# HuiGuanLab/Lite-MKD

Hardware: AMD Instinct MI355X
Metric: episodes/sec (5-way 5-shot, 8x224^2 frames) (higher is better)
Workload: dtype f32

## Files before the change

### include/lmkd.h

```cpp
#ifndef LMKD_H
#define LMKD_H
#ifdef __cplusplus
extern "C" {
#endif

int lmkd_abi_version(void);
const char* lmkd_last_error(void);
int lmkd_device_check(int device);
int lmkd_set_activation_dtype(int mode);
int lmkd_get_activation_dtype(void);

int lmkd_gemm_f32(char layA, char layB, int M, int N, int K, float alpha, const float* A, long lda, long sA,
                  const float* B, long ldb, long sB, float beta, float* C, long ldc, long sC, const float* bias,
                  int relu, int batch, void* stream);
int lmkd_gemm_set_mode(int mode);
int lmkd_gemm_set_tile(int t);
long lmkd_gemm_ticket_words(void);
int lmkd_gemm_f32_splitk(char layA, char layB, int M, int N, int K, float alpha, const float* A, long lda, long sA,
                         const float* B, long ldb, long sB, float beta, float* C, long ldc, long sC, const float* bias,
                         int relu, int batch, void* workspace, long ws_bytes, unsigned* tickets, void* stream);

long lmkd_conv2d_packed_weight_elems(int Cout, int Cin, int Cs, int KH, int KW, int mode);
int lmkd_conv2d_pack_weights(const float* w_oihw, float* wp, int Cout, int Cin, int Cs, int KH, int KW, int mode ,
                             void* stream);
// ... 175 lines not shown

int lmkd_conv2d_fwd_row_tiles_seg(int N, int H, int W, int Cs, int Cout, int KH, int KW, int stride, int pad, int seg_n0, int* tiles0 );
int lmkd_conv2d_fwd_seg(const float* x, const float* pre_stats , const float* wp, float* y,
                        float* stat_partial, int N, int H, int W, int Cs, int Cout, int KH, int KW, int stride, int pad, int seg_n0, void* stream,
                        const lmkd_amax_desc* amax );
int lmkd_conv2d_bwd_data_bn_tiles_seg(int N, int H, int W, int Cin, int Cout, int KH, int KW, int stride, int pad, int seg_n0, int* tiles0 );
int lmkd_conv2d_bwd_data_seg(const float* dy, const float* wd, float* dx, const float* bn_x ,
                             const float* bn_stats, float* part, int N, int H, int W, int Cin, int Cout, int KH, int KW, int stride, int pad,
                             int accumulate, int seg_n0, void* stream, const lmkd_amax_desc* amax );
long lmkd_conv2d_bwd_weight_workspace_seg(int N, int H, int W, int Cs, int Cout, int KH, int KW, int stride, int pad, int seg_n0);
int lmkd_conv2d_bwd_weight_seg(const float* x, const float* pre_stats , const float* dy, float* dw_oihw, float* workspace,
                               long ws_bytes, int N, int H, int W, int Cs, int Cin, int Cout, int KH, int KW, int stride, int pad, int accumulate,
                               int seg_n0, void* stream, const lmkd_amax_desc* amax );
int lmkd_bn_finalize_seg(const float* partial, int T, int T0, int C, long count0, long count1, const float* gamma, const float* beta, float eps,
                         float* stats , double* scratch, unsigned* tickets, void* stream, const lmkd_amax_desc* amax );
int lmkd_bn_apply_seg(const float* x, const float* stats, const float* res, const float* rstats, float* y, long rows, long rows0, int C, int relu,
                      int res_mode, unsigned* mask_bits, void* stream, const lmkd_amax_desc* amax );
int lmkd_bn_backward_seg(const float* dy, const float* x, const float* yact, const float* stats, const float* gamma, float* dx, float* g_out,
                         float* dgamma, float* dbeta, float* coef, void* workspace, unsigned* tickets, long rows, long rows0, int C, int mask_mode,
                         int accumulate_param_grads, void* stream, const lmkd_amax_desc* amax );
int lmkd_bn_backward_part_seg(const float* part, int T, int T0, const float* dy, const float* x, const float* stats, const float* gamma, float* dx,
                              float* dgamma, float* dbeta, float* coef, void* workspace, unsigned* tickets, long rows, long rows0, int C,
                              int accumulate_param_grads, void* stream, const lmkd_amax_desc* amax );
int lmkd_bn_relu_maxpool_fwd_seg(const float* x, const float* stats, float* y, unsigned char* idx, float* cmax, int N, int N0, int H, int W, int C,
                                 void* stream, const lmkd_amax_desc* amax );
int lmkd_bn_backward_stats_seg(const float* dy, const float* cmax, const float* stats, const float* gamma, float* coef, void* workspace,
                               unsigned* tickets, long pooled_rows, long pooled_rows0, long count, long count0, int C, void* stream);
int lmkd_stem_unpool_bn_bwd_seg(const float* dy, const unsigned char* idx, const float* c, const float* stats, const float* coef, float* dc,
                                float* dgamma, float* dbeta, int accumulate_param_grads, int N, int N0, int H, int W, int C, void* stream,
                                const lmkd_amax_desc* amax );

int lmkd_strm_patchpool_fwd(const float* x, const float* pe, const float* mask, float* y, unsigned char* idx, int F, int H, int W, int C,
                            void* stream);
int lmkd_strm_patchpool_bwd(const float* dy, const float* mask, const unsigned char* idx, float* dx, int F, int H, int W, int C, void* stream);
int lmkd_strm_attn_fwd(const float* x, const float* qkv, const float* gamma, float* y, float* probs, int F, int C, void* stream);
int lmkd_strm_attn_bwd(const float* dy, const float* qkv, const float* probs, const float* gamma, float* dqkv, float* dgamma_part,
                       float* dgamma, int F, int C, void* stream);
long lmkd_strm_tokmlp_parts(long V, int D);
int lmkd_strm_tokmlp_fwd(const float* x, const float* pe, const float* mask, const float* w1, const float* b1, const float* w2, const float* b2,
                         float* xp, float* y, unsigned char* hmask, int V, int L, int D, void* stream);
int lmkd_strm_tokmlp_bwd(const float* dy, const float* xp, const float* mask, const float* w1, const float* b1, const float* w2, float* dx,
                         float* part, float* dparams, int V, int L, int D, void* stream);
int lmkd_strm_pair_embed(const float* P, const float* bias, float* E, int NV, int L, int Hd, void* stream);
int lmkd_strm_patchdist_fwd(const float* E, const int* order, float* dist, int* idx, float* logits, int Ns, int Nq, int way, int shot, int L,
                            int Hd, void* stream);
int lmkd_strm_patchdist_bwd(const float* E, const int* order, const int* pos, const float* dist, const int* idx, const float* g, float* dpre,
// ... 7 lines not shown
```

### lite-mkd_amd/csrc/norm_pool.hip

```cpp
#include "common.h"
#include <vector>
#include <cmath>
#include <algorithm>

#define NP_THREADS 256
static int g_ew_wg_per_cu = 4;
extern "C" int lmkd_set_elementwise_wg_per_cu(int n) {
  LMKD_REQUIRE(n >= 1 && n <= 8, "lmkd_set_elementwise_wg_per_cu: %d outside 1..8 (the BatchNorm partial buffers hold 2048 rows)", n);
  g_ew_wg_per_cu = n;
  return LMKD_OK;
}
static inline int ew_grid(long n_items) {
  long g = (n_items + NP_THREADS - 1) / NP_THREADS;
  if (g > 256 * g_ew_wg_per_cu) g = 256 * g_ew_wg_per_cu;
  if (g < 1) g = 1;
  return (int)g;
}

extern "C" long lmkd_amax_words(void) { return 2 * LMKD_AMAX_SEG_WORDS; }
static inline unsigned* amd_out(const lmkd_amax_desc* d) { return d ? (unsigned*)d->out_words : nullptr; }
static inline const unsigned* amd_ref(const lmkd_amax_desc* d) { return (d && d->out_words) ? (const unsigned*)d->ref_words : nullptr; }

#define LMKD_FENCE_MAX 128
struct FenceArgs { const unsigned* w[LMKD_FENCE_MAX]; unsigned* r[LMKD_FENCE_MAX]; };
// ... 591 lines not shown
      const float4 g = bn_masked_grad<T>(dv[u], xv[u], yact, i0 + u, stats, C, c + 4 * u, mask_mode);
      s1[u].x += g.x; s1[u].y += g.y; s1[u].z += g.z; s1[u].w += g.w;
      s2[u].x = fmaf(g.x, (xv[u].x - mean[u].x) * istd[u].x, s2[u].x); s2[u].y = fmaf(g.y, (xv[u].y - mean[u].y) * istd[u].y, s2[u].y);
      s2[u].z = fmaf(g.z, (xv[u].z - mean[u].z) * istd[u].z, s2[u].z); s2[u].w = fmaf(g.w, (xv[u].w - mean[u].w) * istd[u].w, s2[u].w);
    }
  }
#pragma unroll
  for (int u = 0; u < U; ++u) {
    float* d = sm + ((long)rl * CC + cq * 4 * U + 4 * u) * 2;
    d[0] = s1[u].x; d[1] = s2[u].x; d[2] = s1[u].y; d[3] = s2[u].y; d[4] = s1[u].z; d[5] = s2[u].z; d[6] = s1[u].w; d[7] = s2[u].w;
  }
  __syncthreads();
  for (int j = threadIdx.x; j < 2 * CC; j += NP_THREADS) {
#pragma unroll
    for (int h = 0; h < U; ++h) {
      if (blockIdx.x * U + h >= nbv) break;
      float s = 0.f;
      for (int q = h * RL1; q < (h + 1) * RL1; ++q) s += sm[(long)q * 2 * CC + j];
      partial[(long)(blockIdx.x * U + h) * 2 * C + 2 * c0 + j] = s;
    }
  }
}

struct CoefSeg { int T1; long pstride; double count1; int S0, S1; };
__global__ void bn_bwd_coef_kernel(const float* __restrict__ part, int T, int C, double count, const float* __restrict__ gamma,
                                   const float* __restrict__ stats, float* __restrict__ coef, float* __restrict__ dgamma,
                                   float* __restrict__ dbeta, int accumulate, double* __restrict__ scratch, unsigned* __restrict__ tickets,
                                   CoefSeg cs) {
  __shared__ double sm[CS_LANES][CS_COLS];
  __shared__ double tot[CS_COLS];
  __shared__ int s_last;
  int S = 0;
  const bool seg = gridDim.z > 1;
  if (seg) {
    if (blockIdx.z) { part += cs.pstride; T = cs.T1; count = cs.count1; stats += 5 * C; coef += 5 * C; scratch += (long)(CS_MAX_SLICES + 2) * 2 * C; tickets += LMKD_TICKET_WORDS / 2; S = cs.S1; }
    else S = cs.S0;
  }
  if (!colsum_ticket(part, T, 2 * C, scratch, tickets, sm, tot, &s_last, nullptr, S)) return;
  const int c = blockIdx.x * (CS_COLS / 2) + threadIdx.x;
  if (threadIdx.y != 0 || threadIdx.x >= CS_COLS / 2 || c >= C) return;
  const double sg = tot[2 * threadIdx.x], sgx = tot[2 * threadIdx.x + 1];
  const float g = gamma ? gamma[c] : 1.f;
  const float invstd = stats[C + c];
  coef[c] = g * invstd;
  coef[C + c] = (float)(sg / count);
  coef[2 * C + c] = (float)(sgx / count);
  if (seg) {
    coef[3 * C + c] = (float)sgx;
    coef[4 * C + c] = (float)sg;
    return;
  }
  if (dgamma) dgamma[c] = accumulate ? dgamma[c] + (float)sgx : (float)sgx;
  if (dbeta) dbeta[c] = accumulate ? dbeta[c] + (float)sg : (float)sg;
}

struct ParamGradSeg { float* dgamma; float* dbeta; int accumulate; };
__device__ __forceinline__ void bn_param_grads_seg(const float* __restrict__ coef, int C, const ParamGradSeg& pg) {
  if (blockIdx.x != 0 || !pg.dgamma) return;
  for (int c = threadIdx.x; c < C; c += blockDim.x) {
    const float gx = coef[3 * C + c] + coef[5 * C + 3 * C + c], g = coef[4 * C + c] + coef[5 * C + 4 * C + c];
    pg.dgamma[c] = pg.accumulate ? pg.dgamma[c] + gx : gx;
    if (pg.dbeta) pg.dbeta[c] = pg.accumulate ? pg.dbeta[c] + g : g;
  }
}

template <typename T>
__global__ void bn_bwd_apply_kernel(const T* __restrict__ dy, const T* __restrict__ x, const T* __restrict__ yact,
                                    const float* __restrict__ stats, const float* __restrict__ coef, T* __restrict__ dx,
                                    T* __restrict__ g_out, long n4, int C, int mask_mode, long n4_0, ParamGradSeg pg,
                                    unsigned* __restrict__ amax, const unsigned* __restrict__ aref) {
  constexpr int U = ActU<T>::U;
  const int C4 = C >> 2;
  const long nu = n4 / U;
  if (n4_0 < n4) bn_param_grads_seg(coef, C, pg);
  AmaxStat am = {0.f, 0.f, 0u}, am1 = {0.f, 0.f, 0u};
  const AmaxRef rf0 = amax_ref(aref ? amax_read(aref, 0) : 0u), rf1 = amax_ref(aref ? amax_read(aref, 1) : 0u);
  for (long iu = (long)blockIdx.x * blockDim.x + threadIdx.x; iu < nu; iu += (long)gridDim.x * blockDim.x) {
    float4 xv[U], dv[U], o[U], gq[U];
    ldv<T, U>(x, iu, xv);
    ldv<T, U>(dy, iu, dv);
    const int so = iu * U >= n4_0 ? 5 * C : 0;
// ... 5 lines not shown
      const int c = (int)(i % C4) * 4;
      const float4 g = bn_masked_grad<T>(dv[u], xv[u], yact, i, st, C, c, mask_mode);
      const float4 mean = *reinterpret_cast<const float4*>(st + c);
      const float4 istd = *reinterpret_cast<const float4*>(st + C + c);
      const float4 A = *reinterpret_cast<const float4*>(cf + c);
      const float4 mg = *reinterpret_cast<const float4*>(cf + C + c);
      const float4 mgx = *reinterpret_cast<const float4*>(cf + 2 * C + c);
      o[u].x = A.x * (g.x - mg.x - (xv[u].x - mean.x) * istd.x * mgx.x);
      o[u].y = A.y * (g.y - mg.y - (xv[u].y - mean.y) * istd.y * mgx.y);
      o[u].z = A.z * (g.z - mg.z - (xv[u].z - mean.z) * istd.z * mgx.z);
      o[u].w = A.w * (g.w - mg.w - (xv[u].w - mean.w) * istd.w * mgx.w);
      gq[u] = g;
      if (so) amax_stat4(am1, o[u], rf1); else amax_stat4(am, o[u], rf0);
    }
    stv<T, U>(dx, iu, o);
    if (g_out) stv<T, U>(g_out, iu, gq);
  }
  if (amax) {
    amax_commit_stat(amax, am, aref != nullptr);
    if (n4_0 < n4) amax_commit_stat(amax + LMKD_AMAX_SEG_WORDS, am1, aref != nullptr);
  }
}

extern "C" long lmkd_bn_bwd_workspace(int C) { return (long)(2048 * 2 * C) * sizeof(float) + (long)(66 * 2 * C) * sizeof(double) + 64; }

static int bn_bwd_stats_impl(const float* dy, const float* x, const float* yact, const float* stats, const float* gamma, float* dgamma,
                             float* dbeta, float* coef, void* workspace, unsigned* tickets, long rows, long count, int C, int mask_mode,
                             int accumulate_param_grads, hipStream_t s, const char* who, long rows0 = 0, long count0 = 0) {
  LMKD_REQUIRE(dy && x && stats && coef && workspace && tickets, "%s: null pointer", who);
  const bool seg = rows0 > 0 && rows0 < rows;
  LMKD_REQUIRE(!seg || cdiv(2 * C, CS_COLS) <= LMKD_TICKET_WORDS / 2, "%s: C=%d exceeds the ticket buffer", who, C);
  const int CC = C > 1024 ? 1024 : C;
  const int U = g_lmkd_act_bf16 ? 2 : 1;
  LMKD_REQUIRE(C % (4 * U) == 0 && C % CC == 0 && 256 % (CC / 4) == 0, "%s: unsupported channel count %d", who, C);
  LMKD_REQUIRE((mask_mode != 1 && mask_mode != 3) || yact, "%s: mask_mode 1 / 3 needs the activation output / its bit mask", who);
  LMKD_REQUIRE(mask_mode != 3 || C % 32 == 0, "%s: bit masks need C %% 32 == 0", who);
  LMKD_REQUIRE(cdiv(2 * C, CS_COLS) <= LMKD_TICKET_WORDS, "%s: C=%d exceeds the ticket buffer", who, C);
  const int RL1 = NP_THREADS / (CC / 4), RL = RL1 * U;
  auto blocks = [&](long r) {
    int nb = cdiv(r, (long)RL1 * 8);
    if (nb > 256 * g_ew_wg_per_cu * 2) nb = 256 * g_ew_wg_per_cu * 2;
    if (nb > 2048) nb = 2048;
    return nb < 1 ? 1 : nb;
  };
  const int nb = blocks(seg ? rows0 : rows), nb1 = seg ? blocks(rows - rows0) : 0;
  const int nbx = std::max(nb, nb1);
  float* partial = (float*)workspace;
  double* dscr = (double*)((char*)workspace + (((long)(seg ? 2 : 1) * 2048 * 2 * C * sizeof(float) + 63) / 64) * 64);
  BnSeg bs;
  bs.rows0 = seg ? rows0 : rows; bs.nb1 = nb1;
  const int gz = seg ? 2 : 1;
  if (g_lmkd_act_bf16)
    hipLaunchKernelGGL(bn_bwd_reduce_kernel<lmkd_bf16_t>, dim3(cdiv(nbx, 2), C / CC, gz), dim3(NP_THREADS), (size_t)RL * CC * 2 * sizeof(float), s,
                       (const lmkd_bf16_t*)dy, (const lmkd_bf16_t*)x, (const lmkd_bf16_t*)yact, stats, partial, rows, C, CC, mask_mode, nb, bs);
  else
    hipLaunchKernelGGL(bn_bwd_reduce_kernel<float>, dim3(nbx, C / CC, gz), dim3(NP_THREADS), (size_t)RL * CC * 2 * sizeof(float), s, dy, x, yact,
                       stats, partial, rows, C, CC, mask_mode, nb, bs);
  LMKD_CHECK_LAUNCH("bn_bwd_reduce_kernel");
  CoefSeg cs;
  cs.T1 = nb1; cs.pstride = (long)2048 * 2 * C; cs.count1 = (double)(count - count0); cs.S0 = cs_slices(nb); cs.S1 = seg ? cs_slices(nb1) : 0;
  hipLaunchKernelGGL(bn_bwd_coef_kernel, dim3(cdiv(2 * C, CS_COLS), std::max(cs.S0, cs.S1), gz), dim3(CS_COLS, CS_LANES), 0, s, (const float*)partial, nb, C,
                     (double)(seg ? count0 : count), gamma, stats, coef, dgamma, dbeta, accumulate_param_grads, dscr, tickets, cs);
  LMKD_CHECK_LAUNCH("bn_bwd_coef_kernel");
  return LMKD_OK;
}

extern "C" int lmkd_bn_backward_seg(const float* dy, const float* x, const float* yact, const float* stats, const float* gamma, float* dx,
                                    float* g_out, float* dgamma, float* dbeta, float* coef, void* workspace, unsigned* tickets, long rows,
                                    long rows0, int C, int mask_mode, int accumulate_param_grads, void* stream, const lmkd_amax_desc* amd);
extern "C" int lmkd_bn_backward(const float* dy, const float* x, const float* yact, const float* stats, const float* gamma,
                                float* dx, float* g_out, float* dgamma, float* dbeta, float* coef, void* workspace, unsigned* tickets,
// ... 2 lines not shown
                              accumulate_param_grads, stream, nullptr);
}
extern "C" int lmkd_bn_backward_seg(const float* dy, const float* x, const float* yact, const float* stats, const float* gamma, float* dx,
                                    float* g_out, float* dgamma, float* dbeta, float* coef, void* workspace, unsigned* tickets, long rows,
                                    long rows0, int C, int mask_mode, int accumulate_param_grads, void* stream, const lmkd_amax_desc* amd) {
  unsigned* amax = amd_out(amd);
  const unsigned* aref = amd_ref(amd);
  LMKD_REQUIRE(dx, "lmkd_bn_backward: null pointer");
  hipStream_t s = (hipStream_t)stream;
  if (rows0 <= 0 || rows0 >= rows) rows0 = rows;
  const int rc = bn_bwd_stats_impl(dy, x, yact, stats, gamma, dgamma, dbeta, coef, workspace, tickets, rows, rows, C, mask_mode,
                                   accumulate_param_grads, s, "lmkd_bn_backward", rows0, rows0);
  if (rc) return rc;
  const long n4 = rows * C / 4, n4_0 = rows0 * C / 4;
  ParamGradSeg pg;
  pg.dgamma = dgamma; pg.dbeta = dbeta; pg.accumulate = accumulate_param_grads;
  if (g_lmkd_act_bf16)
    hipLaunchKernelGGL(bn_bwd_apply_kernel<lmkd_bf16_t>, dim3(ew_grid(n4)), dim3(NP_THREADS), 0, s, (const lmkd_bf16_t*)dy, (const lmkd_bf16_t*)x,
                       (const lmkd_bf16_t*)yact, stats, (const float*)coef, (lmkd_bf16_t*)dx, (lmkd_bf16_t*)g_out, n4, C, mask_mode, n4_0, pg, amax, aref);
  else
    hipLaunchKernelGGL(bn_bwd_apply_kernel<float>, dim3(ew_grid(n4)), dim3(NP_THREADS), 0, s, dy, x, yact, stats, (const float*)coef, dx, g_out,
                       n4, C, mask_mode, n4_0, pg, amax, aref);
  LMKD_CHECK_LAUNCH("bn_bwd_apply_kernel");
  return LMKD_OK;
}

extern "C" int lmkd_bn_backward_part_seg(const float* part, int T, int T0, const float* dy, const float* x, const float* stats, const float* gamma,
                                         float* dx, float* dgamma, float* dbeta, float* coef, void* workspace, unsigned* tickets, long rows,
                                         long rows0, int C, int accumulate_param_grads, void* stream, const lmkd_amax_desc* amd);
extern "C" int lmkd_bn_backward_part(const float* part, int T, const float* dy, const float* x, const float* stats, const float* gamma,
                                     float* dx, float* dgamma, float* dbeta, float* coef, void* workspace, unsigned* tickets, long rows, int C,
                                     int accumulate_param_grads, void* stream) {
  return lmkd_bn_backward_part_seg(part, T, T, dy, x, stats, gamma, dx, dgamma, dbeta, coef, workspace, tickets, rows, rows, C,
                                   accumulate_param_grads, stream, nullptr);
}
extern "C" int lmkd_bn_backward_part_seg(const float* part, int T, int T0, const float* dy, const float* x, const float* stats, const float* gamma,
                                         float* dx, float* dgamma, float* dbeta, float* coef, void* workspace, unsigned* tickets, long rows,
                                         long rows0, int C, int accumulate_param_grads, void* stream, const lmkd_amax_desc* amd) {
  unsigned* amax = amd_out(amd);
  const unsigned* aref = amd_ref(amd);
  LMKD_REQUIRE(part && T > 0 && dy && x && stats && dx && coef && workspace && tickets, "lmkd_bn_backward_part: null pointer");
  LMKD_REQUIRE(!g_lmkd_act_bf16 && C % 4 == 0, "lmkd_bn_backward_part: fp32 tensors, C %% 4 == 0");
  const bool seg = T0 > 0 && T0 < T && rows0 > 0 && rows0 < rows;
  LMKD_REQUIRE(seg || (T0 == T && rows0 == rows), "lmkd_bn_backward_part_seg: T0 / rows0 must both name a split or both the whole");
  LMKD_REQUIRE(cdiv(2 * C, CS_COLS) <= LMKD_TICKET_WORDS / (seg ? 2 : 1), "lmkd_bn_backward_part: C=%d exceeds the ticket buffer", C);
  hipStream_t s = (hipStream_t)stream;
// ... 401 lines not shown
```

### lite-mkd_amd/ops.py

```python
import ctypes
import os
import math

import torch

from ._lib import lib
from . import _audit


def _raw_stream(device_index=None):
    return torch._C._cuda_getCurrentRawStream(torch._C._cuda_getDevice() if device_index is None else device_index)


def _stream():
    return ctypes.c_void_p(_raw_stream())


def _p(t):
    if t is None:
        return None
    if _audit.ON:
        _audit.note(t)
    return ctypes.c_void_p(t.data_ptr())

# ... 81 lines not shown
        e = _GEMM_WS[key] = (torch.empty(32 << 20, dtype=torch.uint8, device=like.device),
                             torch.zeros(lib().value("lmkd_gemm_ticket_words"), dtype=torch.int32, device=like.device))
    return e


def stack_rows(a, b):
    if (a.dim() == 2 and b.dim() == 2 and a.shape[1] == b.shape[1] and a.dtype == b.dtype and a.is_contiguous() and b.is_contiguous()
            and a.numel() > 0 and b.numel() > 0 and a.untyped_storage().data_ptr() == b.untyped_storage().data_ptr()
            and a.storage_offset() + a.numel() == b.storage_offset()):
        return torch.as_strided(a, (a.shape[0] + b.shape[0], a.shape[1]), (a.shape[1], 1), a.storage_offset())
    return torch.cat([a, b], 0)


def linear_fwd(x, w, b):
    M, K = x.shape
    N = w.shape[0]
    y = _empty((M, N), x)
    return gemm("K", "K", M, N, K, x, K, w, K, y, N, bias=b)


_TICKETS = {}


def _tickets(like):
    key = (like.device.index, _raw_stream(like.device.index))
    t = _TICKETS.get(key)
    if t is None:
        t = _TICKETS[key] = torch.zeros(lib().value("lmkd_ticket_words"), dtype=torch.int32, device=like.device)
    return t


def colsum(a, b=None, out=None, accumulate=False):
    rows, C = a.shape
    if out is None:
        out = _empty((C,), a)
        accumulate = False
    _chk(a, b, out)
    ws = torch.empty(lib().value("lmkd_colsum_workspace", C), dtype=torch.uint8, device=a.device)
    lib().call("lmkd_colsum", _p(a), _p(b), _p(out), rows, C, int(accumulate), _p(ws), _p(_tickets(a)), _stream())
    return out


DIRECT_PARAM_GRAD = False
_GRAD_SLOT = {}


def register_grad_slot(param, shadow_view):
    _GRAD_SLOT[param.data_ptr()] = (weakref.ref(param), shadow_view)
# ... 756 lines not shown
    rows = x.numel() // C
    seg = _seg_frames(seg, x.shape[0])
    rows0 = _rows0(x, seg)
    _chk(dy, x, yact, stats, gamma)
    dx = dx_out if dx_out is not None else torch.empty_like(x)
    g = torch.empty_like(x) if want_g else None
    tg = _grad_target(gamma) if beta is not None else None
    tb = _grad_target(beta) if tg is not None else None
    direct = tg is not None and tb is not None
    dgamma, dbeta = (tg, tb) if direct else (_empty((C,), x), _empty((C,), x))
    coef = _empty((2, 5, C) if seg else (3, C), x)
    ws = torch.empty(lib().value("lmkd_bn_bwd_workspace", C) * (2 if seg else 1), dtype=torch.uint8, device=x.device)
    if part is not None:
        if mask_mode != 2 or want_g:
            raise ValueError("partial sums of the data gradient: mask_mode 2 without g")
        part, T0 = part if isinstance(part, tuple) else (part, part.shape[0])
        _chk(part)
        lib().call("lmkd_bn_backward_part_seg", _p(part), part.shape[0], T0, _p(dy), _p(x), _p(stats), _p(gamma), _p(dx), _p(dgamma), _p(dbeta),
                   _p(coef), _p(ws), _p(_tickets(x)), rows, rows0, C, int(direct), _stream(), _desc_arg(_amax_out(dx, ("d", gamma.data_ptr()))))
    else:
        lib().call("lmkd_bn_backward_seg", _p(dy), _p(x), _p(yact), _p(stats), _p(gamma), _p(dx), _p(g), _p(dgamma), _p(dbeta),
                   _p(coef), _p(ws), _p(_tickets(x)), rows, rows0, C, mask_mode, int(direct), _stream(), _desc_arg(_amax_out(dx, ("d", gamma.data_ptr()))))
    return (dx, g, None, None) if direct else (dx, g, dgamma, dbeta)


_DEFER = None


def set_defer(lst):
    global _DEFER
    _DEFER = lst


def deferring():
    return _DEFER is not None


def apply_deferred(entries, counters=None):
    if not entries:
        return
    layers, order = {}, []
    for rm, rv, stats in entries:
        k = rm.data_ptr()
        if k not in layers:
            layers[k] = [rm, rv, []]
            order.append(k)
# ... 607 lines not shown
        ctx.stride = stride
        ctx.has_ds = wd is not None
        ctx.fused = fused
        ctx.betas = (b1, b2, bd)
        if BLOCK_TAPS is not None:
            BLOCK_TAPS.append({"c1": c1, "st1": st1, "y": y, "seg": seg})
        if training:
            ctx.save_for_backward(x, w1, g1, c1, st1, a1, w2, g2, c2, st2, ybits if fused else y, wd, gd, cd, std)
            ctx.amax = (_amax_tag(x), _amax_tag(a1), _amax_tag(c1))
        return y

    @staticmethod
    def backward(ctx, dy):
        _audit.engine_owned(dy)
        if not ctx.training:
            raise NotImplementedError("backward through eval-mode BatchNorm is not part of the hot path")
        x, w1, g1, c1, st1, a1, w2, g2, c2, st2, y, wd, gd, cd, std = ctx.saved_tensors
        for t, tag in zip((x, a1, c1), ctx.amax):
            _amax_retag(t, tag)
        dy = dy.contiguous()
        stride = ctx.stride
        seg = ctx.seg
        Cmid = w1.shape[0]
        dc2, g, dg2, db2 = bn_backward(dy, c2, y, st2, g2, 3 if ctx.fused else 1, want_g=True, beta=ctx.betas[1], seg=seg)
        wd2 = pack_weights(w2, Cmid, 1)
        dw2 = weight_grad(w2, c1, dc2, 1, 1, st1, seg=seg) if a1 is None else weight_grad(w2, a1, dc2, 1, 1, seg=seg)
        da1, part1 = conv_bwd_data(dc2, wd2, c1.shape, Cmid, 3, 3, 1, 1, bn=(c1, st1), seg=seg)
        del dc2
        dc1, _, dg1, db1 = bn_backward(da1, c1, None, st1, g1, 2, dx_out=da1, beta=ctx.betas[0], part=part1, seg=seg)
        dw1 = weight_grad(w1, x, dc1, stride, 1, seg=seg)
        dwd = dgd = dbd = None
        need_dx = ctx.needs_input_grad[0]
        dx = None
        if ctx.has_ds:
            dcd, _, dgd, dbd = bn_backward(g, cd, None, std, gd, 0, dx_out=g, beta=ctx.betas[2], seg=seg)
            dwd = weight_grad(wd, x, dcd, stride, 0, seg=seg)
            if need_dx:
                dx = conv_bwd_data(dc1, pack_weights(w1, Cmid, 1), x.shape, Cmid, 3, 3, stride, 1, seg=seg)
                conv_bwd_data(dcd, pack_weights(wd, Cmid, 1), x.shape, Cmid, 1, 1, stride, 0, out=dx, accumulate=True, seg=seg)
        else:
            dx = g
            if need_dx:
                conv_bwd_data(dc1, pack_weights(w1, Cmid, 1), x.shape, Cmid, 3, 3, stride, 1, out=dx, accumulate=True, seg=seg)
        return (dx if need_dx else None, None, None, dw1, dg1, db1, None, None, dw2, dg2, db2, None, None,
                dwd, dgd, dbd, None, None, None)


class BottleneckFn(torch.autograd.Function):

    @staticmethod
    def forward(ctx, x, stride, training, w1, g1, b1, rm1, rv1, w2, g2, b2, rm2, rv2, w3, g3, b3, rm3, rv3,
                wd, gd, bd, rmd, rvd, seg=0):
        _chk(x, w1, w2, w3, wd)
        Cs = x.shape[-1]
        Cm = w1.shape[0]
        if not training and _eval_fused():
            ctx.training = False
            a1 = conv_bn_eval(x, w1, Cs, 1, 0, g1, b1, rm1, rv1, True)
# ... 1122 lines not shown
```

### lite-mkd_amd/schedule.py

```python
import contextlib
import dataclasses
import os


_PIPELINE = [False]


@dataclasses.dataclass
class Schedule:
    conv_dtype: str = "fp32x3"
    act_dtype: str = "fp32"
    overlap_trunk_calls: bool = True
    merge_trunk_calls: bool = False
    pipeline_episodes: bool = False
    side_wgrad: bool = True
    sync_wgrad_at_backward_end: bool = False
    teacher_stream: bool = True
    heads_on_two_streams: bool = True
    side_linear_wgrad: bool = True
    direct_param_grad: bool = True
    repack_at_step: bool = True
    fuse_two_head_linear: bool = True
    dgrad_bn_stats: bool = True
    stem_pooled_bwd: bool = True
    pre_in_plane_modes: bool = True
    fuse_pre_all_modes: bool = False
    trx_proj_on_conv: bool = False
    gemm_split_k: bool = False

    @classmethod
    def bench(cls, **over):
        kw = dict(merge_trunk_calls=True, pipeline_episodes=True)
        kw.update(over)
        return cls(**kw)

    @classmethod
    def two_call(cls, **over):
        return cls(**over)

    @classmethod
    def serial(cls, **over):
        kw = dict(overlap_trunk_calls=False, merge_trunk_calls=False, side_wgrad=False, sync_wgrad_at_backward_end=True, teacher_stream=False,
                  heads_on_two_streams=False, side_linear_wgrad=False, direct_param_grad=False, repack_at_step=False, pipeline_episodes=False)
        kw.update(over)
        return cls(**kw)

    @classmethod
    def from_env(cls, env=None, **over):
        env = os.environ if env is None else env
        names = {"overlap_trunk_calls": "LMKD_OVERLAP", "merge_trunk_calls": "LMKD_MERGE", "pipeline_episodes": "LMKD_PIPELINE", "side_wgrad": "LMKD_SIDE_WGRAD",
                 "sync_wgrad_at_backward_end": "LMKD_SYNC_WG", "teacher_stream": "LMKD_TEACHER_STREAM", "heads_on_two_streams": "LMKD_HEADS2",
                 "side_linear_wgrad": "LMKD_SIDE_LINEAR", "direct_param_grad": "LMKD_DIRECT_GRAD", "repack_at_step": "LMKD_REPACK",
                 "fuse_two_head_linear": "LMKD_FC_FUSED", "dgrad_bn_stats": "LMKD_DGRAD_BN", "stem_pooled_bwd": "LMKD_STEM_POOLED",
                 "pre_in_plane_modes": "LMKD_PRE_X3", "fuse_pre_all_modes": "LMKD_FUSE_PRE", "trx_proj_on_conv": "LMKD_TRX_CONV",
                 "gemm_split_k": "LMKD_GEMM_SPLIT"}
        s = cls.bench(**over)
        for field, var in names.items():
            if var in env and field not in over:
                setattr(s, field, env[var] == "1")
        return s

    _WHERE = {
        "overlap_trunk_calls": ("model.backbone.resnet", "OVERLAP_TRUNK_CALLS"), "merge_trunk_calls": ("model.backbone.resnet", "MERGE_TRUNK_CALLS"),
        "side_wgrad": ("ops", "SIDE_WGRAD"), "sync_wgrad_at_backward_end": ("ops", "SYNC_WGRAD_AT_BACKWARD_END"),
        "teacher_stream": ("trainloop", "TEACHER_STREAM"), "heads_on_two_streams": ("ops", "HEADS_ON_TWO_STREAMS"),
        "side_linear_wgrad": ("ops", "SIDE_LINEAR_WGRAD"), "direct_param_grad": ("ops", "DIRECT_PARAM_GRAD"),
        "repack_at_step": ("trainloop", "REPACK_AT_STEP"), "fuse_two_head_linear": ("ops", "FUSE_TWO_HEAD_LINEAR"),
        "dgrad_bn_stats": ("ops", "DGRAD_BN_STATS"), "stem_pooled_bwd": ("ops", "STEM_POOLED_BWD"),
        "pre_in_plane_modes": ("ops", "PRE_IN_PLANE_MODES"), "fuse_pre_all_modes": ("ops", "FUSE_PRE_ALL_MODES"),
        "trx_proj_on_conv": ("ops", "TRX_PROJ_ON_CONV"), "gemm_split_k": ("ops", "GEMM_SPLIT_K"),
    }

    def _targets(self):
        import importlib
        pkg = __name__.rsplit(".", 1)[0]
        for field, (mod, attr) in self._WHERE.items():
            yield field, importlib.import_module(pkg + "." + mod), attr

    def apply(self, arithmetic=True):
        from . import ops
        for field, mod, attr in self._targets():
            setattr(mod, attr, bool(getattr(self, field)))
        _PIPELINE[0] = bool(self.pipeline_episodes)
        if arithmetic:
            ops.set_conv_compute_dtype(self.conv_dtype)
            ops.set_activation_dtype(self.act_dtype)
        return self

    @classmethod
    def current(cls):
        from . import ops
        s = cls(conv_dtype=ops.get_conv_compute_dtype(), act_dtype=ops.get_activation_dtype(), pipeline_episodes=_PIPELINE[0])
        for field, mod, attr in s._targets():
# ... 15 lines not shown
```

Baseline: 50.73.

## Fuse main and downsample BatchNorm backward passes in residual block into one dual kernel set

Adds a dual BatchNorm backward path that handles the main branch's second BN and the downsample BN together, since both consume the same upstream gradient. One reduce kernel reads dy and the mask once and accumulates statistics for both sides, one coef kernel finalizes both, and one apply kernel writes both dx tensors. This removes a separate three-kernel sequence and a second pass over dy. The cost is extra per-side workspace, a second ticket slot per stream, more register pressure in the fused kernels, and a fallback to the old path when only one side has direct parameter-grad targets.

New measurement: 50.91, median of 6. No clear change (+0.4%).

```diff
diff --git a/include/lmkd.h b/include/lmkd.h
--- a/include/lmkd.h
+++ b/include/lmkd.h
@@ -221,6 +221,12 @@
 int lmkd_bn_backward_part_seg(const float* part, int T, int T0, const float* dy, const float* x, const float* stats, const float* gamma, float* dx,
                               float* dgamma, float* dbeta, float* coef, void* workspace, unsigned* tickets, long rows, long rows0, int C,
                               int accumulate_param_grads, void* stream, const lmkd_amax_desc* amax );
+int lmkd_bn_backward_dual_seg(const float* dy, const float* yact, const float* x_a, const float* stats_a, const float* gamma_a, float* dx_a,
+                              float* dgamma_a, float* dbeta_a, float* coef_a, void* workspace_a, unsigned* tickets_a,
+                              const lmkd_amax_desc* amax_a , const float* x_b, const float* stats_b, const float* gamma_b,
+                              float* dx_b, float* dgamma_b, float* dbeta_b, float* coef_b, void* workspace_b, unsigned* tickets_b,
+                              const lmkd_amax_desc* amax_b , long rows, long rows0, int C, int mask_mode,
+                              int accumulate_param_grads, void* stream);
 int lmkd_bn_relu_maxpool_fwd_seg(const float* x, const float* stats, float* y, unsigned char* idx, float* cmax, int N, int N0, int H, int W, int C,
                                  void* stream, const lmkd_amax_desc* amax );
 int lmkd_bn_backward_stats_seg(const float* dy, const float* cmax, const float* stats, const float* gamma, float* coef, void* workspace,
diff --git a/lite-mkd_amd/csrc/norm_pool.hip b/lite-mkd_amd/csrc/norm_pool.hip
--- a/lite-mkd_amd/csrc/norm_pool.hip
+++ b/lite-mkd_amd/csrc/norm_pool.hip
@@ -637,18 +637,88 @@
   }
 }
 
+template <typename T>
+__global__ void bn_bwd_reduce_dual_kernel(const T* __restrict__ dy, const T* __restrict__ xa, const T* __restrict__ xb,
+                                          const T* __restrict__ yact, const float* __restrict__ stats_a, const float* __restrict__ stats_b,
+                                          float* __restrict__ partial_a, float* __restrict__ partial_b, long rows, int C, int CC,
+                                          int mask_mode, int nbv, BnSeg sg) {
+  extern __shared__ float sm[];
+  constexpr int U = ActU<T>::U;
+  if (gridDim.z > 1) {
+    if (blockIdx.z) {
+      const long eo = sg.rows0 * C;
+      dy += eo; xa += eo; xb += eo;
+      if (yact) yact = mask_mode == 3 ? reinterpret_cast<const T*>(reinterpret_cast<const unsigned*>(yact) + eo / 32) : yact + eo;
+      stats_a += 5 * C; stats_b += 5 * C; partial_a += (long)2048 * 2 * C; partial_b += (long)2048 * 2 * C; rows -= sg.rows0; nbv = sg.nb1;
+    } else {
+      rows = sg.rows0;
+    }
+  }
+  const int C4 = C >> 2, CCV = CC / (4 * U);
+  const int RL = NP_THREADS / CCV, RL1 = RL / U;
+  const int cq = threadIdx.x % CCV, rl = threadIdx.x / CCV;
+  const int bv = blockIdx.x * U + rl / RL1, vl = rl % RL1;
+  const int c0 = blockIdx.y * CC;
+  const int c = c0 + cq * 4 * U;
+  float4 s1[U], s2a[U], s2b[U], mean_a[U], istd_a[U], mean_b[U], istd_b[U];
+#pragma unroll
+  for (int u = 0; u < U; ++u) {
+    s1[u] = make_float4(0, 0, 0, 0); s2a[u] = make_float4(0, 0, 0, 0); s2b[u] = make_float4(0, 0, 0, 0);
+    mean_a[u] = *reinterpret_cast<const float4*>(stats_a + c + 4 * u);
+    istd_a[u] = *reinterpret_cast<const float4*>(stats_a + C + c + 4 * u);
+    mean_b[u] = *reinterpret_cast<const float4*>(stats_b + c + 4 * u);
+    istd_b[u] = *reinterpret_cast<const float4*>(stats_b + C + c + 4 * u);
+  }
+  for (long r = bv < nbv ? (long)bv * RL1 + vl : rows; r < rows; r += (long)nbv * RL1) {
+    const long i0 = r * C4 + (c >> 2);
+    float4 xv[U], xw[U], dv[U];
+    ldv<T, U>(xa, i0 / U, xv);
+    ldv<T, U>(xb, i0 / U, xw);
+    ldv<T, U>(dy, i0 / U, dv);
+#pragma unroll
+    for (int u = 0; u < U; ++u) {
+      const float4 g = bn_masked_grad<T>(dv[u], xv[u], yact, i0 + u, stats_a, C, c + 4 * u, mask_mode);
+      s1[u].x += g.x; s1[u].y += g.y; s1[u].z += g.z; s1[u].w += g.w;
+      s2a[u].x = fmaf(g.x, (xv[u].x - mean_a[u].x) * istd_a[u].x, s2a[u].x); s2a[u].y = fmaf(g.y, (xv[u].y - mean_a[u].y) * istd_a[u].y, s2a[u].y);
+      s2a[u].z = fmaf(g.z, (xv[u].z - mean_a[u].z) * istd_a[u].z, s2a[u].z); s2a[u].w = fmaf(g.w, (xv[u].w - mean_a[u].w) * istd_a[u].w, s2a[u].w);
+      s2b[u].x = fmaf(g.x, (xw[u].x - mean_b[u].x) * istd_b[u].x, s2b[u].x); s2b[u].y = fmaf(g.y, (xw[u].y - mean_b[u].y) * istd_b[u].y, s2b[u].y);
+      s2b[u].z = fmaf(g.z, (xw[u].z - mean_b[u].z) * istd_b[u].z, s2b[u].z); s2b[u].w = fmaf(g.w, (xw[u].w - mean_b[u].w) * istd_b[u].w, s2b[u].w);
+    }
+  }
+#pragma unroll
+  for (int side = 0; side < 2; ++side) {
+    if (side) __syncthreads();
+#pragma unroll
+    for (int u = 0; u < U; ++u) {
+      const float4 s2 = side ? s2b[u] : s2a[u];
+      float* d = sm + ((long)rl * CC + cq * 4 * U + 4 * u) * 2;
+      d[0] = s1[u].x; d[1] = s2.x; d[2] = s1[u].y; d[3] = s2.y; d[4] = s1[u].z; d[5] = s2.z; d[6] = s1[u].w; d[7] = s2.w;
+    }
+    __syncthreads();
+    float* partial = side ? partial_b : partial_a;
+    for (int j = threadIdx.x; j < 2 * CC; j += NP_THREADS) {
+#pragma unroll
+      for (int h = 0; h < U; ++h) {
+        if (blockIdx.x * U + h >= nbv) break;
+        float s = 0.f;
+        for (int q = h * RL1; q < (h + 1) * RL1; ++q) s += sm[(long)q * 2 * CC + j];
+        partial[(long)(blockIdx.x * U + h) * 2 * C + 2 * c0 + j] = s;
+      }
+    }
+  }
+}
+
 struct CoefSeg { int T1; long pstride; double count1; int S0, S1; };
-__global__ void bn_bwd_coef_kernel(const float* __restrict__ part, int T, int C, double count, const float* __restrict__ gamma,
-                                   const float* __restrict__ stats, float* __restrict__ coef, float* __restrict__ dgamma,
-                                   float* __restrict__ dbeta, int accumulate, double* __restrict__ scratch, unsigned* __restrict__ tickets,
-                                   CoefSeg cs) {
+__device__ __forceinline__ void bn_bwd_coef_body(const float* __restrict__ part, int T, int C, double count, const float* __restrict__ gamma,
+                                                 const float* __restrict__ stats, float* __restrict__ coef, float* __restrict__ dgamma,
+                                                 float* __restrict__ dbeta, int accumulate, double* __restrict__ scratch,
+                                                 unsigned* __restrict__ tickets, const CoefSeg& cs, bool seg, int z) {
   __shared__ double sm[CS_LANES][CS_COLS];
   __shared__ double tot[CS_COLS];
   __shared__ int s_last;
   int S = 0;
-  const bool seg = gridDim.z > 1;
   if (seg) {
-    if (blockIdx.z) { part += cs.pstride; T = cs.T1; count = cs.count1; stats += 5 * C; coef += 5 * C; scratch += (long)(CS_MAX_SLICES + 2) * 2 * C; tickets += LMKD_TICKET_WORDS / 2; S = cs.S1; }
+    if (z) { part += cs.pstride; T = cs.T1; count = cs.count1; stats += 5 * C; coef += 5 * C; scratch += (long)(CS_MAX_SLICES + 2) * 2 * C; tickets += LMKD_TICKET_WORDS / 2; S = cs.S1; }
     else S = cs.S0;
   }
   if (!colsum_ticket(part, T, 2 * C, scratch, tickets, sm, tot, &s_last, nullptr, S)) return;
@@ -668,10 +738,23 @@
   if (dgamma) dgamma[c] = accumulate ? dgamma[c] + (float)sgx : (float)sgx;
   if (dbeta) dbeta[c] = accumulate ? dbeta[c] + (float)sg : (float)sg;
 }
+__global__ void bn_bwd_coef_kernel(const float* __restrict__ part, int T, int C, double count, const float* __restrict__ gamma,
+                                   const float* __restrict__ stats, float* __restrict__ coef, float* __restrict__ dgamma,
+                                   float* __restrict__ dbeta, int accumulate, double* __restrict__ scratch, unsigned* __restrict__ tickets,
+                                   CoefSeg cs) {
+  bn_bwd_coef_body(part, T, C, count, gamma, stats, coef, dgamma, dbeta, accumulate, scratch, tickets, cs, gridDim.z > 1, blockIdx.z);
+}
+struct CoefSide { const float* part; const float* gamma; const float* stats; float* coef; float* dgamma; float* dbeta; double* scratch; unsigned* tickets; };
+__global__ void bn_bwd_coef_dual_kernel(CoefSide a, CoefSide b, int T, int C, double count, int accumulate, CoefSeg cs, int seg) {
+  const int side = seg ? blockIdx.z >> 1 : blockIdx.z;
+  bn_bwd_coef_body(side ? b.part : a.part, T, C, count, side ? b.gamma : a.gamma, side ? b.stats : a.stats, side ? b.coef : a.coef,
+                   side ? b.dgamma : a.dgamma, side ? b.dbeta : a.dbeta, accumulate, side ? b.scratch : a.scratch,
+                   side ? b.tickets : a.tickets, cs, seg != 0, seg ? blockIdx.z & 1 : 0);
+}
 
 struct ParamGradSeg { float* dgamma; float* dbeta; int accumulate; };
-__device__ __forceinline__ void bn_param_grads_seg(const float* __restrict__ coef, int C, const ParamGradSeg& pg) {
-  if (blockIdx.x != 0 || !pg.dgamma) return;
+__device__ __forceinline__ void bn_param_grads_seg(const float* __restrict__ coef, int C, const ParamGradSeg& pg, unsigned blk = 0u) {
+  if (blockIdx.x != blk || !pg.dgamma) return;
   for (int c = threadIdx.x; c < C; c += blockDim.x) {
     const float gx = coef[3 * C + c] + coef[5 * C + 3 * C + c], g = coef[4 * C + c] + coef[5 * C + 4 * C + c];
     pg.dgamma[c] = pg.accumulate ? pg.dgamma[c] + gx : gx;
@@ -723,12 +806,73 @@
   }
 }
 
+__device__ __forceinline__ float4 bn_bwd_dx4(const float4 g, const float4 xv, const float* __restrict__ st, const float* __restrict__ cf,
+                                             int C, int c) {
+  const float4 mean = *reinterpret_cast<const float4*>(st + c);
+  const float4 istd = *reinterpret_cast<const float4*>(st + C + c);
+  const float4 A = *reinterpret_cast<const float4*>(cf + c);
+  const float4 mg = *reinterpret_cast<const float4*>(cf + C + c);
+  const float4 mgx = *reinterpret_cast<const float4*>(cf + 2 * C + c);
+  float4 o;
+  o.x = A.x * (g.x - mg.x - (xv.x - mean.x) * istd.x * mgx.x);
+  o.y = A.y * (g.y - mg.y - (xv.y - mean.y) * istd.y * mgx.y);
+  o.z = A.z * (g.z - mg.z - (xv.z - mean.z) * istd.z * mgx.z);
+  o.w = A.w * (g.w - mg.w - (xv.w - mean.w) * istd.w * mgx.w);
+  return o;
+}
+
+struct ApplySide { const float* stats; const float* coef; ParamGradSeg pg; unsigned* amax; const unsigned* aref; };
+template <typename T>
+__global__ void bn_bwd_apply_dual_kernel(const T* __restrict__ dy, const T* __restrict__ yact, const T* __restrict__ xa,
+                                         const T* __restrict__ xb, T* __restrict__ dxa, T* __restrict__ dxb, ApplySide sa, ApplySide sb,
+                                         long n4, int C, int mask_mode, long n4_0) {
+  constexpr int U = ActU<T>::U;
+  const int C4 = C >> 2;
+  const long nu = n4 / U;
+  if (n4_0 < n4) {
+    bn_param_grads_seg(sa.coef, C, sa.pg);
+    bn_param_grads_seg(sb.coef, C, sb.pg, gridDim.x > 1 ? 1u : 0u);
+  }
+  AmaxStat ama = {0.f, 0.f, 0u}, ama1 = {0.f, 0.f, 0u}, amb = {0.f, 0.f, 0u}, amb1 = {0.f, 0.f, 0u};
+  const AmaxRef ra0 = amax_ref(sa.aref ? amax_read(sa.aref, 0) : 0u), ra1 = amax_ref(sa.aref ? amax_read(sa.aref, 1) : 0u);
+  const AmaxRef rb0 = amax_ref(sb.aref ? amax_read(sb.aref, 0) : 0u), rb1 = amax_ref(sb.aref ? amax_read(sb.aref, 1) : 0u);
+  for (long iu = (long)blockIdx.x * blockDim.x + threadIdx.x; iu < nu; iu += (long)gridDim.x * blockDim.x) {
+    float4 xv[U], xw[U], dv[U], oa[U], ob[U];
+    ldv<T, U>(xa, iu, xv);
+    ldv<T, U>(xb, iu, xw);
+    ldv<T, U>(dy, iu, dv);
+    const int so = iu * U >= n4_0 ? 5 * C : 0;
+#pragma unroll
+    for (int u = 0; u < U; ++u) {
+      const long i = iu * U + u;
+      const int c = (int)(i % C4) * 4;
+      const float4 g = bn_masked_grad<T>(dv[u], xv[u], yact, i, sa.stats + so, C, c, mask_mode);
+      oa[u] = bn_bwd_dx4(g, xv[u], sa.stats + so, sa.coef + so, C, c);
+      ob[u] = bn_bwd_dx4(g, xw[u], sb.stats + so, sb.coef + so, C, c);
+      if (so) { amax_stat4(ama1, oa[u], ra1); amax_stat4(amb1, ob[u], rb1); }
+      else { amax_stat4(ama, oa[u], ra0); amax_stat4(amb, ob[u], rb0); }
+    }
+    stv<T, U>(dxa, iu, oa);
+    stv<T, U>(dxb, iu, ob);
+  }
+  if (sa.amax) {
+    amax_commit_stat(sa.amax, ama, sa.aref != nullptr);
+    if (n4_0 < n4) amax_commit_stat(sa.amax + LMKD_AMAX_SEG_WORDS, ama1, sa.aref != nullptr);
+  }
+  if (sb.amax) {
+    amax_commit_stat(sb.amax, amb, sb.aref != nullptr);
+    if (n4_0 < n4) amax_commit_stat(sb.amax + LMKD_AMAX_SEG_WORDS, amb1, sb.aref != nullptr);
+  }
+}
+
 extern "C" long lmkd_bn_bwd_workspace(int C) { return (long)(2048 * 2 * C) * sizeof(float) + (long)(66 * 2 * C) * sizeof(double) + 64; }
 
-static int bn_bwd_stats_impl(const float* dy, const float* x, const float* yact, const float* stats, const float* gamma, float* dgamma,
-                             float* dbeta, float* coef, void* workspace, unsigned* tickets, long rows, long count, int C, int mask_mode,
-                             int accumulate_param_grads, hipStream_t s, const char* who, long rows0 = 0, long count0 = 0) {
-  LMKD_REQUIRE(dy && x && stats && coef && workspace && tickets, "%s: null pointer", who);
+struct BnBwdPlan {
+  bool seg;
+  int C, CC, U, RL1, RL, nb, nb1;
+  double* scratch(void* workspace) const { return (double*)((char*)workspace + (((long)(seg ? 2 : 1) * 2048 * 2 * C * sizeof(float) + 63) / 64) * 64); }
+};
+static int bn_bwd_plan(BnBwdPlan& p, const void* yact, long rows, long rows0, int C, int mask_mode, const char* who) {
   const bool seg = rows0 > 0 && rows0 < rows;
   LMKD_REQUIRE(!seg || cdiv(2 * C, CS_COLS) <= LMKD_TICKET_WORDS / 2, "%s: C=%d exceeds the ticket buffer", who, C);
   const int CC = C > 1024 ? 1024 : C;
@@ -744,10 +888,22 @@
     if (nb > 2048) nb = 2048;
     return nb < 1 ? 1 : nb;
   };
-  const int nb = blocks(seg ? rows0 : rows), nb1 = seg ? blocks(rows - rows0) : 0;
-  const int nbx = std::max(nb, nb1);
+  p.seg = seg; p.C = C; p.CC = CC; p.U = U; p.RL1 = RL1; p.RL = RL;
+  p.nb = blocks(seg ? rows0 : rows); p.nb1 = seg ? blocks(rows - rows0) : 0;
+  return LMKD_OK;
+}
+
+static int bn_bwd_stats_impl(const float* dy, const float* x, const float* yact, const float* stats, const float* gamma, float* dgamma,
+                             float* dbeta, float* coef, void* workspace, unsigned* tickets, long rows, long count, int C, int mask_mode,
+                             int accumulate_param_grads, hipStream_t s, const char* who, long rows0 = 0, long count0 = 0) {
+  LMKD_REQUIRE(dy && x && stats && coef && workspace && tickets, "%s: null pointer", who);
+  BnBwdPlan p;
+  const int prc = bn_bwd_plan(p, yact, rows, rows0, C, mask_mode, who);
+  if (prc) return prc;
+  const bool seg = p.seg;
+  const int CC = p.CC, RL = p.RL, nb = p.nb, nb1 = p.nb1, nbx = std::max(nb, nb1);
   float* partial = (float*)workspace;
-  double* dscr = (double*)((char*)workspace + (((long)(seg ? 2 : 1) * 2048 * 2 * C * sizeof(float) + 63) / 64) * 64);
+  double* dscr = p.scratch(workspace);
   BnSeg bs;
   bs.rows0 = seg ? rows0 : rows; bs.nb1 = nb1;
   const int gz = seg ? 2 : 1;
@@ -796,6 +952,57 @@
     hipLaunchKernelGGL(bn_bwd_apply_kernel<float>, dim3(ew_grid(n4)), dim3(NP_THREADS), 0, s, dy, x, yact, stats, (const float*)coef, dx, g_out,
                        n4, C, mask_mode, n4_0, pg, amax, aref);
   LMKD_CHECK_LAUNCH("bn_bwd_apply_kernel");
+  return LMKD_OK;
+}
+
+extern "C" int lmkd_bn_backward_dual_seg(const float* dy, const float* yact, const float* x_a, const float* stats_a, const float* gamma_a,
+                                         float* dx_a, float* dgamma_a, float* dbeta_a, float* coef_a, void* workspace_a,
+                                         unsigned* tickets_a, const lmkd_amax_desc* amd_a, const float* x_b, const float* stats_b,
+                                         const float* gamma_b, float* dx_b, float* dgamma_b, float* dbeta_b, float* coef_b,
+                                         void* workspace_b, unsigned* tickets_b, const lmkd_amax_desc* amd_b, long rows, long rows0, int C,
+                                         int mask_mode, int accumulate_param_grads, void* stream) {
+  const char* who = "lmkd_bn_backward_dual_seg";
+  LMKD_REQUIRE(dy && x_a && stats_a && dx_a && coef_a && workspace_a && tickets_a && x_b && stats_b && dx_b && coef_b && workspace_b && tickets_b,
+               "%s: null pointer", who);
+  LMKD_REQUIRE(rows > 0 && (mask_mode == 0 || mask_mode == 1 || mask_mode == 3), "%s: mask_mode 0, 1 or 3 (got %d)", who, mask_mode);
+  LMKD_REQUIRE(workspace_a != workspace_b && tickets_a != tickets_b && coef_a != coef_b && dx_a != dx_b, "%s: the two sides share a buffer", who);
+  LMKD_REQUIRE((const float*)dx_a != dy && (const float*)dx_b != dy, "%s: dx must not alias dy", who);
+  hipStream_t s = (hipStream_t)stream;
+  if (rows0 <= 0 || rows0 >= rows) rows0 = rows;
+  BnBwdPlan p;
+  const int prc = bn_bwd_plan(p, yact, rows, rows0, C, mask_mode, who);
+  if (prc) return prc;
+  const bool seg = p.seg;
+  const int nbx = std::max(p.nb, p.nb1), gz = seg ? 2 : 1;
+  BnSeg bs;
+  bs.rows0 = rows0; bs.nb1 = p.nb1;
+  const size_t lds = (size_t)p.RL * p.CC * 2 * sizeof(float);
+  if (g_lmkd_act_bf16)
+    hipLaunchKernelGGL(bn_bwd_reduce_dual_kernel<lmkd_bf16_t>, dim3(cdiv(nbx, 2), C / p.CC, gz), dim3(NP_THREADS), lds, s, (const lmkd_bf16_t*)dy,
+                       (const lmkd_bf16_t*)x_a, (const lmkd_bf16_t*)x_b, (const lmkd_bf16_t*)yact, stats_a, stats_b, (float*)workspace_a,
+                       (float*)workspace_b, rows, C, p.CC, mask_mode, p.nb, bs);
+  else
+    hipLaunchKernelGGL(bn_bwd_reduce_dual_kernel<float>, dim3(nbx, C / p.CC, gz), dim3(NP_THREADS), lds, s, dy, x_a, x_b, yact, stats_a, stats_b,
+                       (float*)workspace_a, (float*)workspace_b, rows, C, p.CC, mask_mode, p.nb, bs);
+  LMKD_CHECK_LAUNCH("bn_bwd_reduce_dual_kernel");
+  CoefSeg cs;
+  cs.T1 = p.nb1; cs.pstride = (long)2048 * 2 * C; cs.count1 = (double)(rows - rows0); cs.S0 = cs_slices(p.nb); cs.S1 = seg ? cs_slices(p.nb1) : 0;
+  CoefSide ca = {(const float*)workspace_a, gamma_a, stats_a, coef_a, dgamma_a, dbeta_a, p.scratch(workspace_a), tickets_a};
+  CoefSide cb = {(const float*)workspace_b, gamma_b, stats_b, coef_b, dgamma_b, dbeta_b, p.scratch(workspace_b), tickets_b};
+  hipLaunchKernelGGL(bn_bwd_coef_dual_kernel, dim3(cdiv(2 * C, CS_COLS), std::max(cs.S0, cs.S1), 2 * gz), dim3(CS_COLS, CS_LANES), 0, s, ca, cb,
+                     p.nb, C, (double)rows0, accumulate_param_grads, cs, seg ? 1 : 0);
+  LMKD_CHECK_LAUNCH("bn_bwd_coef_dual_kernel");
+  const long n4 = rows * C / 4, n4_0 = rows0 * C / 4;
+  ApplySide aa = {stats_a, coef_a, {dgamma_a, dbeta_a, accumulate_param_grads}, amd_out(amd_a), amd_ref(amd_a)};
+  ApplySide ab = {stats_b, coef_b, {dgamma_b, dbeta_b, accumulate_param_grads}, amd_out(amd_b), amd_ref(amd_b)};
+  if (g_lmkd_act_bf16)
+    hipLaunchKernelGGL(bn_bwd_apply_dual_kernel<lmkd_bf16_t>, dim3(ew_grid(n4)), dim3(NP_THREADS), 0, s, (const lmkd_bf16_t*)dy,
+                       (const lmkd_bf16_t*)yact, (const lmkd_bf16_t*)x_a, (const lmkd_bf16_t*)x_b, (lmkd_bf16_t*)dx_a, (lmkd_bf16_t*)dx_b, aa, ab,
+                       n4, C, mask_mode, n4_0);
+  else
+    hipLaunchKernelGGL(bn_bwd_apply_dual_kernel<float>, dim3(ew_grid(n4)), dim3(NP_THREADS), 0, s, dy, yact, x_a, x_b, dx_a, dx_b, aa, ab, n4, C,
+                       mask_mode, n4_0);
+  LMKD_CHECK_LAUNCH("bn_bwd_apply_dual_kernel");
   return LMKD_OK;
 }
 
diff --git a/lite-mkd_amd/ops.py b/lite-mkd_amd/ops.py
--- a/lite-mkd_amd/ops.py
+++ b/lite-mkd_amd/ops.py
@@ -127,8 +127,8 @@
 _TICKETS = {}
 
 
-def _tickets(like):
-    key = (like.device.index, _raw_stream(like.device.index))
+def _tickets(like, slot=0):
+    key = (like.device.index, _raw_stream(like.device.index)) + ((slot,) if slot else ())
     t = _TICKETS.get(key)
     if t is None:
         t = _TICKETS[key] = torch.zeros(lib().value("lmkd_ticket_words"), dtype=torch.int32, device=like.device)
@@ -931,6 +931,40 @@
         lib().call("lmkd_bn_backward_seg", _p(dy), _p(x), _p(yact), _p(stats), _p(gamma), _p(dx), _p(g), _p(dgamma), _p(dbeta),
                    _p(coef), _p(ws), _p(_tickets(x)), rows, rows0, C, mask_mode, int(direct), _stream(), _desc_arg(_amax_out(dx, ("d", gamma.data_ptr()))))
     return (dx, g, None, None) if direct else (dx, g, dgamma, dbeta)
+
+
+BN_DUAL = True
+
+
+def bn_backward_dual(dy, yact, mask_mode, xa, stats_a, gamma_a, beta_a, xb, stats_b, gamma_b, beta_b, seg=0):
+    C = xa.shape[-1]
+    rows = xa.numel() // C
+    seg = _seg_frames(seg, xa.shape[0])
+    rows0 = _rows0(xa, seg)
+    if xb.shape != xa.shape or dy.shape != xa.shape:
+        raise ValueError("bn_backward_dual: dy and both BatchNorm inputs must have one shape")
+    _chk(dy, yact, xa, stats_a, gamma_a, xb, stats_b, gamma_b)
+    targets = []
+    for gamma, beta in ((gamma_a, beta_a), (gamma_b, beta_b)):
+        tg = _grad_target(gamma) if beta is not None else None
+        tb = _grad_target(beta) if tg is not None else None
+        targets.append((tg, tb) if tg is not None and tb is not None else None)
+    if (targets[0] is None) != (targets[1] is None):
+        return None
+    direct = targets[0] is not None
+    sides = []
+    for slot, (x, gamma) in enumerate(((xa, gamma_a), (xb, gamma_b))):
+        dx = torch.empty_like(x)
+        tg, tb = targets[slot] if direct else (_empty((C,), x), _empty((C,), x))
+        sides.append({"dx": dx, "tg": tg, "tb": tb, "coef": _empty((2, 5, C) if seg else (3, C), x),
+                      "ws": torch.empty(lib().value("lmkd_bn_bwd_workspace", C) * (2 if seg else 1), dtype=torch.uint8, device=x.device),
+                      "tickets": _tickets(x, slot), "desc": _amax_out(dx, ("d", gamma.data_ptr()))})
+    a, b = sides
+    lib().call("lmkd_bn_backward_dual_seg", _p(dy), _p(yact),
+               _p(xa), _p(stats_a), _p(gamma_a), _p(a["dx"]), _p(a["tg"]), _p(a["tb"]), _p(a["coef"]), _p(a["ws"]), _p(a["tickets"]), _desc_arg(a["desc"]),
+               _p(xb), _p(stats_b), _p(gamma_b), _p(b["dx"]), _p(b["tg"]), _p(b["tb"]), _p(b["coef"]), _p(b["ws"]), _p(b["tickets"]), _desc_arg(b["desc"]),
+               rows, rows0, C, mask_mode, int(direct), _stream())
+    return tuple((sd["dx"], None, None) if direct else (sd["dx"], sd["tg"], sd["tb"]) for sd in sides)
 
 
 _DEFER = None
@@ -1584,18 +1618,25 @@
         stride = ctx.stride
         seg = ctx.seg
         Cmid = w1.shape[0]
-        dc2, g, dg2, db2 = bn_backward(dy, c2, y, st2, g2, 3 if ctx.fused else 1, want_g=True, beta=ctx.betas[1], seg=seg)
+        dual = dgd = dbd = None
+        if ctx.has_ds and BN_DUAL:
+            dual = bn_backward_dual(dy, y, 3 if ctx.fused else 1, c2, st2, g2, ctx.betas[1], cd, std, gd, ctx.betas[2], seg=seg)
+        if dual is not None:
+            (dc2, dg2, db2), (dcd, dgd, dbd) = dual
+        else:
+            dc2, g, dg2, db2 = bn_backward(dy, c2, y, st2, g2, 3 if ctx.fused else 1, want_g=True, beta=ctx.betas[1], seg=seg)
         wd2 = pack_weights(w2, Cmid, 1)
         dw2 = weight_grad(w2, c1, dc2, 1, 1, st1, seg=seg) if a1 is None else weight_grad(w2, a1, dc2, 1, 1, seg=seg)
         da1, part1 = conv_bwd_data(dc2, wd2, c1.shape, Cmid, 3, 3, 1, 1, bn=(c1, st1), seg=seg)
         del dc2
         dc1, _, dg1, db1 = bn_backward(da1, c1, None, st1, g1, 2, dx_out=da1, beta=ctx.betas[0], part=part1, seg=seg)
         dw1 = weight_grad(w1, x, dc1, stride, 1, seg=seg)
-        dwd = dgd = dbd = None
+        dwd = None
         need_dx = ctx.needs_input_grad[0]
         dx = None
         if ctx.has_ds:
-            dcd, _, dgd, dbd = bn_backward(g, cd, None, std, gd, 0, dx_out=g, beta=ctx.betas[2], seg=seg)
+            if dual is None:
+                dcd, _, dgd, dbd = bn_backward(g, cd, None, std, gd, 0, dx_out=g, beta=ctx.betas[2], seg=seg)
             dwd = weight_grad(wd, x, dcd, stride, 0, seg=seg)
             if need_dx:
                 dx = conv_bwd_data(dc1, pack_weights(w1, Cmid, 1), x.shape, Cmid, 3, 3, stride, 1, seg=seg)
diff --git a/lite-mkd_amd/schedule.py b/lite-mkd_amd/schedule.py
--- a/lite-mkd_amd/schedule.py
+++ b/lite-mkd_amd/schedule.py
@@ -23,6 +23,7 @@
     fuse_two_head_linear: bool = True
     dgrad_bn_stats: bool = True
     stem_pooled_bwd: bool = True
+    bn_dual: bool = True
     pre_in_plane_modes: bool = True
     fuse_pre_all_modes: bool = False
     trx_proj_on_conv: bool = False
@@ -53,7 +54,7 @@
                  "side_linear_wgrad": "LMKD_SIDE_LINEAR", "direct_param_grad": "LMKD_DIRECT_GRAD", "repack_at_step": "LMKD_REPACK",
                  "fuse_two_head_linear": "LMKD_FC_FUSED", "dgrad_bn_stats": "LMKD_DGRAD_BN", "stem_pooled_bwd": "LMKD_STEM_POOLED",
                  "pre_in_plane_modes": "LMKD_PRE_X3", "fuse_pre_all_modes": "LMKD_FUSE_PRE", "trx_proj_on_conv": "LMKD_TRX_CONV",
-                 "gemm_split_k": "LMKD_GEMM_SPLIT"}
+                 "gemm_split_k": "LMKD_GEMM_SPLIT", "bn_dual": "LMKD_BN_DUAL"}
         s = cls.bench(**over)
         for field, var in names.items():
             if var in env and field not in over:
@@ -69,6 +70,7 @@
         "dgrad_bn_stats": ("ops", "DGRAD_BN_STATS"), "stem_pooled_bwd": ("ops", "STEM_POOLED_BWD"),
         "pre_in_plane_modes": ("ops", "PRE_IN_PLANE_MODES"), "fuse_pre_all_modes": ("ops", "FUSE_PRE_ALL_MODES"),
         "trx_proj_on_conv": ("ops", "TRX_PROJ_ON_CONV"), "gemm_split_k": ("ops", "GEMM_SPLIT_K"),
+        "bn_dual": ("ops", "BN_DUAL"),
     }
 
     def _targets(self):
```
